# author-hidden-name/GAN-segmentation

Hardware: AMD Instinct MI355X
Metric: synthetic (image,mask) pairs/sec, FFHQ-1024 StyleGAN+decoder (higher is better)
Workload: dtype f32; 1 GPU; stylegan-ffhq 1024^2 synthesis + 2-class decoder, batch=8 per GPU, fp32 (BASELINE.json configs[1]); synthetic weights/latents/noise; (img u8, mask u8) resident on rank 0; global_batch=8, parallelism=dp1, gather=none, backend=none, graph=eager (GSA_GRAPH=0)

## Files before the change

### gan-segmentation_amd/csrc/gsa_api.cpp

```cpp
#include <hip/hip_runtime.h>

#include <cmath>
#include <cstdarg>
#include <cstdio>
#include <cstdlib>
#include <cstring>
#include <map>
#include <string>
#include <vector>

#include "../../include/gsa.h"
#include "gsa_kernels.h"
#include "gsa_pack.h"

using namespace gsa;

namespace {

constexpr int kMaxLevels = 12;
thread_local std::string g_create_error;

struct HostTensor {
    std::vector<float> data;
    std::vector<int64_t> dims;
// ... 213 lines not shown
}

bool known_generator_name(const gsa_ctx* c, const char* name) {
    int R = 0, k = 0, i = 0;
    char tail[64], t2[64];
    if (!strcmp(name, "constant_tensor") || !strcmp(name, "latent_avg") || !strcmp(name, "truncation_psi")) return true;
    if (sscanf(name, "mp_dense_%d_%63s", &i, tail) == 2)
        return i >= 0 && i < 8 && (!strcmp(tail, "weight") || !strcmp(tail, "bias") || !strcmp(tail, "std"));
    if (sscanf(name, "%d_%63s", &R, tail) != 2) return false;
    int r = 0;
    while ((1 << r) < R) ++r;
    if ((1 << r) != R || r < 2 || r > c->gc.max_res_log2) return false;
    if (!strcmp(tail, "conv_1_weight") || !strcmp(tail, "conv_1_std")) return r > 2 && r < 7;
    if (!strcmp(tail, "deconv_1_weight") || !strcmp(tail, "deconv_1_std")) return r >= 7;
    if (!strcmp(tail, "blur_1_w_kernel")) return r > 2;
    if (!strcmp(tail, "conv_2_weight") || !strcmp(tail, "conv_2_std")) return true;
    if (!strcmp(tail, "conv_to_rgb_weight") || !strcmp(tail, "conv_to_rgb_bias") || !strcmp(tail, "conv_to_rgb_std"))
        return r == c->gc.max_res_log2;
    if (sscanf(tail, "noise_%d_%63s", &k, t2) == 2) return (k == 1 || k == 2) && !strcmp(t2, "scale_factors");
    if (sscanf(tail, "bias_%d_%63s", &k, t2) == 2) return (k == 1 || k == 2) && !strcmp(t2, "bias");
    if (sscanf(tail, "adain_%d_%63s", &k, t2) == 2)
        return (k == 1 || k == 2) &&
               (!strcmp(t2, "dense_affine_weight") || !strcmp(t2, "dense_affine_bias") || !strcmp(t2, "dense_affine_std") ||
                !strcmp(t2, "norm_gamma") || !strcmp(t2, "norm_beta"));
    return false;
}

int set_param(gsa_ctx* c, std::map<std::string, HostTensor>& m, const char* name, const float* data, int ndim,
              const int64_t* dims) {
    if (!name || !data || ndim < 0 || ndim > 8) return fail(c, GSA_ERR_INVALID, "bad parameter tensor %s", name ? name : "(null)");
    HostTensor t;
    size_t cnt = 1;
    for (int i = 0; i < ndim; ++i) {
        if (dims[i] < 0) return fail(c, GSA_ERR_INVALID, "negative dimension in %s", name);
        t.dims.push_back(dims[i]);
        cnt *= (size_t)dims[i];
    }
    t.data.assign(data, data + cnt);
    m[name] = std::move(t);
    return GSA_OK;
}


struct Launch {
    gsa_ctx* c;
    hipStream_t s;
    const char* label;
    double flops, bytes, alg;
    std::string entry_layer;
    hipEvent_t a = nullptr;
    Launch(gsa_ctx* ctx, hipStream_t st, const char* layer, double flops_, double bytes_, double alg_ = -1.0)
        : c(ctx), s(st), label(layer), flops(flops_), bytes(bytes_), alg(alg_ < 0 ? flops_ : alg_) {
        (void)take_launch_record();
        if (!c->prof) return;
        if (c->prof > 1 && layer) entry_layer = layer;
        if (c->bf16 && layer && strncmp(layer, "g.mapping", 9) && strncmp(layer, "g.styles", 8) && !strstr(layer, "finalize")) bytes *= 0.5;
        a = event();
        (void)hipEventRecord(a, s);
    }
    hipEvent_t event() {
        if (c->event_pool.empty()) {
            hipEvent_t e = nullptr;
            (void)hipEventCreate(&e);
            return e;
        }
        hipEvent_t e = c->event_pool.back();
        c->event_pool.pop_back();
        return e;
    }
    ~Launch() {
        const LaunchRecord r = take_launch_record();
#ifdef GSA_STAMP
        const std::string kname_s = r.count == 1 ? kernel_name(r.kern) : std::string();
        const char* kname = kname_s.c_str();
        if (c->stamps && label && (strstr(kname, "conv") || strstr(kname, "subpixel"))) {
            (void)hipStreamSynchronize(s);
            unsigned long long h[16];
            (void)hipMemcpy(h, c->stamps, sizeof h, hipMemcpyDeviceToHost);
            (void)hipMemset(c->stamps, 0, sizeof h);
            if (h[15] && strstr(kname, "_ws")) {
                const double w = (double)h[15];
                fprintf(stderr, "STAMPWS %-24s %-16s waves %6llu  mfma: work %9.0f barrier %9.0f | mem: write %9.0f load %9.0f epi %9.0f barrier %9.0f\n",
                        kname, label, h[15], h[0] / w, h[1] / w, h[2] / w, h[3] / w, h[4] / w, h[5] / w);
            } else if (h[15] && h[8]) {
                const double w = (double)h[12];
                fprintf(stderr, "STAMPDB %-70s %-14s waves %6llu items/wave %5.1f | per item: write %6.0f load %6.0f (epi-loads %5.0f index %5.0f bulk %5.0f) mfma %6.0f epi %6.0f barrier %6.0f\n",
                        kname, label, h[15], h[12] / (double)h[15], h[6] / w, h[7] / w, h[0] / w, h[1] / w, h[2] / w, h[8] / w, h[9] / w, h[10] / w);
                if (strstr(kname, "subpixel"))
                    fprintf(stderr, "STAMPSW %-14s barrier by wave: %6.0f %6.0f %6.0f %6.0f | write wave0 %6.0f wave3 %6.0f\n", label, 4 * h[0] / w, 4 * h[1] / w, 4 * h[2] / w, 4 * h[3] / w, 4 * h[4] / w, 4 * h[5] / w);
            } else if (h[15]) {
                const double w = (double)h[15];
                fprintf(stderr, "STAMP %-40s %-16s waves %8llu  load %7.0f  write %6.0f  bar %6.0f  blocks %8.0f  epi %7.0f\n", kname,
                        label, h[15], h[0] / w, h[1] / w, h[2] / w, h[3] / w, h[4] / w);
            }
        }
#endif
        if (!a) return;
        if (r.count != 1) {
            c->event_pool.push_back(a);
            if (r.count > 1) ++c->prof_multi;
            return;
        }
        int entry = -1;
        for (size_t i = 0; i < c->prof_entries.size() && entry < 0; ++i)
            if (c->prof_entries[i].kern == r.kern && c->prof_entries[i].layer == entry_layer) entry = (int)i;
        if (entry < 0) {
            ProfEntry e;
            e.kern = r.kern;
            e.layer = entry_layer;
            c->prof_entries.push_back(e);
            entry = (int)c->prof_entries.size() - 1;
        }
        ProfEntry& e = c->prof_entries[entry];
        e.flops += flops;
        e.alg_flops += alg;
        e.bytes += bytes;
        e.launches += 1;
        hipEvent_t b = event();
        (void)hipEventRecord(b, s);
        c->prof_events.push_back(ProfEvent{a, b, entry});
    }
};

}


extern "C" {

#define GSA_STR2(x) #x
#define GSA_STR(x) GSA_STR2(x)
const char* gsa_version(void) {
#ifndef GSA_EXPERIMENTS
#define GSA_EXPERIMENTS 0
#endif
    return "gsa-hip 0.5"
#if GSA_EXPERIMENTS
           "+experiments"
#endif
           " (gfx950, v_mfma_f32_16x16x4_f32 implicit-GEMM convs; built with hipcc = clang " __clang_version__
           ", HIP " GSA_STR(HIP_VERSION_MAJOR) "." GSA_STR(HIP_VERSION_MINOR) "." GSA_STR(HIP_VERSION_PATCH) ")";
}

int gsa_create(int device, gsa_ctx** out) {
    if (!out) return fail(nullptr, GSA_ERR_INVALID, "gsa_create: out is null");
    int count = 0;
    hipError_t e = hipGetDeviceCount(&count);
    if (e != hipSuccess || count <= 0)
        return fail(nullptr, GSA_ERR_HIP, "no HIP device available (%s)", e == hipSuccess ? "device count is 0" : hipGetErrorString(e));
    if (device < 0 || device >= count) return fail(nullptr, GSA_ERR_INVALID, "device %d out of range (%d devices)", device, count);
    e = hipSetDevice(device);
    if (e != hipSuccess) return fail(nullptr, GSA_ERR_HIP, "hipSetDevice(%d): %s", device, hipGetErrorString(e));
    gsa_ctx* c = new gsa_ctx();
    c->device = device;
    e = hipStreamCreateWithFlags(&c->side, hipStreamNonBlocking);
    for (int i = 0; e == hipSuccess && i < kMaxLevels; ++i) e = hipEventCreateWithFlags(&c->ev_level[i], hipEventDisableTiming);
    if (e == hipSuccess) e = hipEventCreateWithFlags(&c->ev_fork, hipEventDisableTiming);
    if (e == hipSuccess) e = hipEventCreateWithFlags(&c->ev_join, hipEventDisableTiming);
    if (e != hipSuccess) {
        const int rc = fail(nullptr, GSA_ERR_HIP, "creating the side stream: %s", hipGetErrorString(e));
        delete c;
        return rc;
    }
    if (e == hipSuccess) e = hipMalloc((void**)&c->zeros, 256);
    if (e == hipSuccess) e = hipMemset(c->zeros, 0, 256);
    if (e != hipSuccess) {
        const int rc = fail(nullptr, GSA_ERR_HIP, "allocating the zero page: %s", hipGetErrorString(e));
// ... 866 lines not shown
```

### gan-segmentation_amd/csrc/gsa_kernels.h

```cpp
#pragma once
#include <hip/hip_runtime.h>
#include <stdint.h>
#include <stdlib.h>

#include <atomic>
#include <string>

namespace gsa {

struct Aff { float mean, A, B, pad; };

struct StatPart { unsigned long long s1, s2; };

constexpr double kStatScale1 = 268435456.0;

enum Epilogue { EPI_RAW = 0, EPI_SYNTH = 1, EPI_DEC = 2 };

struct ConvParams {
    int device;
    const float* src0; const Aff* aff0; int C0;
    const float* src1; int C1;
    int Hs, Ws;
    int up;
    int H, W;
    const float* wpk;
    const float* wino;
    int Cout;
    float* out;
    const float* noise; const float* nscale; const float* nbias;
    StatPart* partials; int prow;
    const float* bn_s; const float* bn_beta;
    const float* resid; int resid_up;
    const float* resid1; int res_c0;
    const float* wsc; const float* sc_bias; float* out_sc;
    int tiles_x, tiles_y, groups, total_tiles;
    int stats_direct;
    int* stat_rows_host;
    int w_resident;
    int group_minor;
    unsigned long long* stamps;
    int dbg;
    int prio;
    int bf16;
    const float* fin_style; int fin_style_stride; const float* fin_gamma; const float* fin_beta; Aff* fin_aff; unsigned* fin_flags;
    const float* zeros;
    const float* rgb_w; const float* rgb_b; uint8_t* rgb_img;
};

struct PostParams {
    const float* src;
    int src_per_sample;
    const float* blur;
    const float* noise; const float* nscale; const float* nbias;
    float* out; StatPart* partials; int prow;
    int H, W, C;
    int bf16;
    int row_groups;
};

struct FinalizeParams {
    const StatPart* partials; int prow; int HW; int C;
    StatPart* acc;
    unsigned* tickets;
    const float* style; int style_stride;
    const float* gamma; const float* beta;
    Aff* aff;
    unsigned* flags;
};

inline int env_int(const char* name, int dflt) {
    const char* v = getenv(name);
    return v ? atoi(v) : dflt;
}


enum class ConvForm { Wino43, WinoDma, WinoTwoTiles, WinoLean, Wino, KSplit, Bf16Lean, Direct };
ConvForm conv3x3_form(const ConvParams& p, int epi, bool shortcut);
hipError_t launch_conv3x3(const ConvParams& p, int epi, bool shortcut, int n, hipStream_t s);
inline bool conv_form_wino(ConvForm f) { return f <= ConvForm::Wino; }
inline double conv_form_products(ConvForm f) { return f == ConvForm::Wino43 ? 2.25 : conv_form_wino(f) ? 4 : 9; }
inline bool wino_shape(int H, int Cout, int bf16) { return !bf16 && (H >= 64 || (H >= 32 && Cout >= 64) || (H >= 16 && Cout >= 256)); }
inline bool wino43_shape(int H, int Cin) { return Cin >= 64 && H >= 32; }
bool wino43_enabled();
bool wino_lean_applies(const ConvParams& p, int epi);
bool wino_stream_paired(const ConvParams& p, int n);
hipError_t launch_wino_lean(const ConvParams& p, int epi, int n, hipStream_t s);
bool wino_lean_fuses_torgb(const ConvParams& p, int epi, int nc);
bool conv_fuses_torgb(const ConvParams& p, int epi, bool shortcut, int nc);
bool bf16_lean_applies(const ConvParams& p, int epi, bool shortcut);
hipError_t launch_bf16_lean(const ConvParams& p, int epi, int n, hipStream_t s);
bool subpixel_lean_applies(const ConvParams& p, int nt, int epi, bool sc, int kb, bool wst);
hipError_t launch_subpixel_lean(const ConvParams& q, int nt, int epi, bool sc, int kb, bool wst, dim3 grid, hipStream_t s);
enum class SubPath { Resident, Streamed, Plain };
struct SubpixelPlan {
    int ct;
    SubPath path;
    bool wino;
    int kb;
    size_t lds;
    int wgs_per_group;
};
SubpixelPlan subpixel_plan(const ConvParams& p, bool shortcut, int n);
hipError_t launch_subpixel(const ConvParams& p, int epi, bool shortcut, int n, hipStream_t s);
bool subpixel_uses_wino(const ConvParams& p);
enum class PostKind { Dma, Packed, Rows, OneRow };
struct PostPlan { PostKind kind; int rpt, row_groups, blocks, rows_used; };
PostPlan post_plan(const PostParams& p);
hipError_t launch_post(const PostParams& p, int n, hipStream_t s);
int post_pk_mode();
bool post_dma_applies(const PostParams& p);
int post_dma_band(const PostParams& p);
int post_dma_blocks(const PostParams& p);
hipError_t launch_post_dma(const PostParams& p, int n, hipStream_t s);
hipError_t launch_post_pk(const PostParams& q, dim3 grid, size_t lds, hipStream_t s);
hipError_t launch_finalize(const FinalizeParams& p, int n, hipStream_t s);
bool conv_fuses_finalize(const ConvParams& p, int epi, bool shortcut);
bool post_fuses_finalize(const PostParams& p);
hipError_t launch_post_fin(const PostParams& p, const FinalizeParams& f, int n, hipStream_t s);
hipError_t launch_pixelnorm(const float* z, float* out, int n, int L, hipStream_t s);
constexpr int kMapSlices = 8;
bool mapping_fused(int L, int device);
hipError_t launch_mapping(const float* z, float* const* wt, float* const* b, unsigned long long* const* ll, float* out, unsigned* ctl,
                          int n, int L, int device, hipStream_t s, int drop_workgroups = 0);
hipError_t launch_dense(const float* x, const float* WT, const float* b, float* y, int n, int K, int J,
                        int lrelu, hipStream_t s);
hipError_t launch_styles(const float* w, const float* avg, const float* psi, const float* WT, const float* b,
                         const int* col_layer, float* styles, int n, int K, int J, hipStream_t s);
hipError_t launch_styles_dlatents(const float* dlatents, const float* avg, const float* psi, const float* WT, const float* b,
                                  const int4* tiles, int num_tiles, float* styles, int n, int K, int J, int NL, hipStream_t s);
hipError_t launch_torgb(const float* x, const Aff* aff, const float* w, const float* b, float* rgb,
                        uint8_t* img, int n, int H, int W, int C, int nc, int bf16, hipStream_t s);
hipError_t launch_torgb_down(const float* x, const Aff* aff, const float* w, const float* b, uint8_t* img, int n, int H, int W, int C,
                             int nc, int f, int bf16, hipStream_t s);
hipError_t launch_final_conv_down(const float* src0, int C0, const float* src1, int C1, const float* wpk, const float* bias, uint8_t* mask,
                                  int n, int H, int W, int ncls, int f, int bf16, hipStream_t s);
hipError_t launch_export_nchw(const float* x, const Aff* aff, float* out, int n, int H, int W, int C, int bf16, hipStream_t s);
hipError_t launch_import_nhwc(const float* in, float* out, int n, int H, int W, int C, int bf16, hipStream_t s);
hipError_t launch_final_conv(const float* src0, int C0, const float* src1, int C1, const float* wpk,
                             const float* bias, float* logits, uint8_t* mask, int n, int H, int W, int ncls, int bf16,
                             hipStream_t s);

int conv_stat_rows(int H, int W, int Cout, int n);
int post_prow(int H, int W, int C);
int post_rows_used(const PostParams& p);
hipError_t launch_fill_normal(float* out, int per_sample, int n, unsigned long long first_index, unsigned plane,
                              unsigned long long seed, hipStream_t s);
hipError_t launch_seg_eval(const float* logits, const int8_t* labels, int n, int classes, int H, int W,
                           unsigned long long* confusion, unsigned long long* loss_fixed, hipStream_t s);

constexpr int kMaxDevices = 64;
int device_cus(int device);
int current_device();
hipError_t allow_max_lds(const void* kern);
hipError_t cached_occupancy(const void* kern, int device, int block, size_t lds, int* wgs_per_cu);
void note_launch(const void* kern);
struct LaunchRecord { const void* kern = nullptr; int count = 0; };
LaunchRecord take_launch_record();
std::string kernel_name(const void* kern);

template <auto K>
hipError_t prepare_kernel(int device) {
    static std::atomic<uint64_t> ready{0};
    if (device < 0 || device >= kMaxDevices) return hipErrorInvalidDevice;
    if (ready.load(std::memory_order_acquire) >> device & 1) return hipSuccess;
    if (hipError_t e = allow_max_lds(reinterpret_cast<const void*>(K))) return e;
    ready.fetch_or(1ull << device, std::memory_order_release);
    return hipSuccess;
}
// ... 17 lines not shown
```

### gan-segmentation_amd/csrc/gsa_wino_lean.hip

```cpp
#include "gsa_kernels.h"
#include "gsa_dev.h"

#include <cstdio>
#include <cstdlib>
#include <type_traits>

namespace gsa {
namespace lean {

constexpr int LH = 18, LW = 18, RS = LW * 16 + 4;
constexpr int IMG = LH * RS;
constexpr int SEG = 16 * 256;
constexpr int NPIX = LH * LW;

struct Tile { int n, y0, x0; };

template <int EPI, bool AFF, bool RES, int NB, int GW, bool DB = true, int PF = 1, bool RGB = false>
__global__ __launch_bounds__(256 * GW, GW == 1 ? (DB ? 2 : 3) : 1) void conv3x3_wino_lean(ConvParams p) {
    static_assert(!RGB || (NB == 1 && GW == 1 && DB && AFF && EPI == EPI_DEC), "fused toRGB: the 16 -> 16 decoder kernel with an AdaIN source");
    static_assert(DB || (NB == 1 && GW == 1), "single-buffered form: one block, one group");
    static_assert(PF == 1 || (PF == 2 && DB), "two prefetch sets: the double-buffered form");
    constexpr int NTHR = 256 * GW, CIN = 16 * NB, COUT = 16 * GW;
    constexpr int NCH = (NPIX * 4 + NTHR - 1) / NTHR;
    constexpr bool kLastPartial = (NPIX * 4) % NTHR != 0;
// ... 297 lines not shown
                epilogue(tc);
                if (EPI == EPI_SYNTH && (!has_next || tr.n != tc.n)) flush_stats(tc.n);
            }
            TICK(k4);
            __syncthreads();
            TICK(k5);
            TSUM(sw, k0, k1); TSUM(sl, k1, k2); TSUM(sm, k2, k3); TSUM(se, k3, k4); TSUM(sb, k4, k5);
            tc = tr; ec = er; cbc = cbr; tr = t2; er = e2c; cbr = cb2; t2 = t3; e2c = e3c; cb2 = cb3;
        };
        for (int it = 0; it < items; it += 2) {
            body(S1{}, it);
            if (it + 1 < items) body(S0{}, it + 1);
        }
        TFLUSH(6, sw); TFLUSH(7, sl); TFLUSH(8, sm); TFLUSH(9, se); TFLUSH(10, sb);
        TFLUSH(12, (unsigned long long)items); TFLUSH(15, 1ull);
        return;
    }
    if (items > 1) { next_item(tr, er, cbr); load_item(S0{}, tr, er, cbr); }
    loads_landed(ra[0]);
    __syncthreads();
    if constexpr (DB) {
        for (int it = 0; it < items; ++it) {
            const bool has_next = it + 1 < items;
            TICK(k0);
            if (has_next) write_item(S0{}, tr, er, cbr, (it + 1) & 1);
            TICK(k1);
            if (cbc == NB - 1) epilogue_loads(tc);
            Tile t2 = tr; int e2c = er, cb2 = cbr;
            if (it + 2 < items) { next_item(t2, e2c, cb2); load_item(S0{}, t2, e2c, cb2); }
            TICK(k2);
            if (NB == 1 || cbc == 0) multiply(std::true_type{}, it & 1, 0);
            else multiply(std::false_type{}, it & 1, cbc);
            loads_landed(ra[0], acc[15]);
            TICK(k3);
            if constexpr (RGB) torgb(tc, it & 1);
            if (cbc == NB - 1) {
                epilogue(tc);
                if (EPI == EPI_SYNTH && (!has_next || tr.n != tc.n)) flush_stats(tc.n);
            }
            TICK(k4);
            __syncthreads();
            TICK(k5);
            TSUM(sw, k0, k1); TSUM(sl, k1, k2); TSUM(sm, k2, k3); TSUM(se, k3, k4); TSUM(sb, k4, k5);
            tc = tr; ec = er; cbc = cbr; tr = t2; er = e2c; cbr = cb2;
        }
        TFLUSH(6, sw); TFLUSH(7, sl); TFLUSH(8, sm); TFLUSH(9, se); TFLUSH(10, sb);
        TFLUSH(12, (unsigned long long)items); TFLUSH(15, 1ull);
    } else {
        for (int it = 0; it < items; ++it) {
            const bool has_next = it + 1 < items;
            transform(0);
            __syncthreads();
            if (has_next) write_item(S0{}, tr, er, 0, 0);
            epilogue_loads(tc);
            Tile t2 = tr; int e2c = er, cb2 = 0;
            if (it + 2 < items) { next_item(t2, e2c, cb2); load_item(S0{}, t2, e2c, cb2); }
            mfmas(std::true_type{}, 0);
            loads_landed(ra[0], acc[15]);
            epilogue(tc);
            if (EPI == EPI_SYNTH && (!has_next || tr.n != tc.n)) flush_stats(tc.n);
            __syncthreads();
            tc = tr; ec = er; tr = t2; er = e2c;
        }
    }
}

__device__ unsigned g_cu_tickets[4096];
__device__ __forceinline__ void antiphase_start(int cycles64, float* lds_word) {
    if (cycles64 <= 0) return;
    if (threadIdx.x == 0) {
        unsigned hw, xcc;
        asm volatile("s_getreg_b32 %0, hwreg(HW_REG_HW_ID)" : "=s"(hw));
        asm volatile("s_getreg_b32 %0, hwreg(HW_REG_XCC_ID)" : "=s"(xcc));
        const unsigned cu = ((xcc & 15u) << 8) | (((hw >> 13) & 7u) << 5) | (((hw >> 12) & 1u) << 4) | ((hw >> 8) & 15u);
        *reinterpret_cast<unsigned*>(lds_word) = atomicAdd(&g_cu_tickets[cu & 4095u], 1u);
    }
    __syncthreads();
    const unsigned ticket = *reinterpret_cast<volatile unsigned*>(lds_word);
    __syncthreads();
    if (ticket & 1u)
        for (int i = 0; i < cycles64; i += 16) __builtin_amdgcn_s_sleep(16);
}

template <int EPI, bool AFF, int NT, int IL, bool PAIR>
__device__ __forceinline__ void wino_stream_body(const ConvParams& p) {
    static_assert(!PAIR || (NT == 1 && IL == 0), "paired form: one group per wave quad, phased memory instructions");
    constexpr int NTHR = PAIR ? 512 : 256;
    constexpr int NCH = (NPIX * 4 + NTHR - 1) / NTHR;
    constexpr int NP = PAIR ? 2 : NT;
    extern __shared__ __attribute__((aligned(16))) float smem[];
    float* const sA = smem;
    float* const sB = smem + 2 * IMG;
    float* const sE = sB + 2 * NP * SEG;
    float* const sC = sE + 64 * NP;
    const int tid = threadIdx.x, lane = tid & 63;
    const int wave8 = __builtin_amdgcn_readfirstlane(tid >> 6);
    const int wave = PAIR ? wave8 & 3 : wave8;
    const int quad = PAIR ? wave8 >> 2 : 0;
    const int i16 = lane & 15, kq = lane >> 4, part = tid & 3;
    const int H = p.H, W = p.W, CIN = p.C0, COUT = p.Cout, nblk = p.C0 >> 4;
    const int g = PAIR ? 2 * (int)blockIdx.y + quad : (int)blockIdx.y;
    const int per = (p.total_tiles + (int)gridDim.x - 1) / (int)gridDim.x;
    const int w_begin = xcd_block(blockIdx.x, gridDim.x) * per;
    const int w_end = min(p.total_tiles, w_begin + per);
    if (w_begin >= w_end) return;
    const int items = (w_end - w_begin) * nblk;
#if GSA_EXPERIMENTS
    antiphase_start(p.group_minor, sC);
#endif

    unsigned s_off[NCH], eflags = 0;
    int l_off[NCH];
#pragma unroll
    for (int k = 0; k < NCH; ++k) {
        const int pix = (tid + NTHR * k) >> 2;
        const bool real = pix < NPIX;
        const int ly = real ? pix / LW : 1, lx = real ? pix % LW : 1;
        s_off[k] = (unsigned)(((ly * W + lx) * CIN + part * 4) * 4);
        l_off[k] = real ? ly * RS + lx * 16 + part * 4 : -1;
        eflags |= (unsigned)((ly == 0 ? 1 : 0) | (ly == LH - 1 ? 2 : 0) | (lx == 0 ? 4 : 0) | (lx == LW - 1 ? 8 : 0)) << (4 * k);
    }
    const unsigned safe_off = (unsigned)((((W + 1) * CIN) + part * 4) * 4);
    auto edge_code = [&](const Tile& t) { return (t.y0 == 0 ? 1 : 0) | (t.y0 + 16 == H ? 2 : 0) | (t.x0 == 0 ? 4 : 0) | (t.x0 + 16 == W ? 8 : 0); };
    auto advance = [&](Tile& t) { t.x0 += 16; if (t.x0 == W) { t.x0 = 0; t.y0 += 16; if (t.y0 == H) { t.y0 = 0; t.n += 1; } } };

    f32x4 ra[NCH];
    int dbg_items = 0; (void)dbg_items;
    const float* const wgrp = p.wpk + (size_t)g * NT * nblk * SEG + lane * 4;
    auto dma_weights = [&](int cb, int buf) {
#ifdef GSA_DBG_HOOKS
        if (p.dbg & 16) cb = 0;
        if ((p.dbg & 1024) && dbg_items > 2) return;
#endif
#pragma unroll
        for (int ct = 0; ct < NT; ++ct) {
            const float* wb = wgrp + ((size_t)ct * nblk + cb) * SEG;
#pragma unroll
            for (int j = 0; j < 4; ++j) {
                const int piece = wave + 4 * j;
                __builtin_amdgcn_global_load_lds((const __attribute__((address_space(1))) void*)(wb + piece * 256),
                                                 (__attribute__((address_space(3))) void*)(sB + (PAIR ? buf * 2 + quad : buf * NT + ct) * SEG + piece * 256), 16, 0, 0);
            }
        }
    };
    auto load_item = [&](const Tile& t, int e, int cb) {
        const char* hb = reinterpret_cast<const char*>(p.src0) + ((((long)(t.n * H + t.y0) * W + t.x0) - (W + 1)) * CIN + cb * 16) * 4;
#ifdef GSA_DBG_HOOKS
        if (p.dbg & 32) hb = reinterpret_cast<const char*>(p.src0) + ((long)(W + 1) * CIN) * 4;
        if ((p.dbg & 512) && dbg_items > 2) return;
#endif
        if (e) {
#pragma unroll
            for (int k = 0; k < NCH; ++k) {
                const unsigned bad = (eflags >> (4 * k)) & (unsigned)e;
                const unsigned off = s_off[k] + (bad ? safe_off - s_off[k] : 0u);
                ra[k] = *reinterpret_cast<const f32x4*>(hb + off);
            }
        } else {
#pragma unroll
            for (int k = 0; k < NCH; ++k) ra[k] = *reinterpret_cast<const f32x4*>(hb + s_off[k]);
        }
    };
    int n_coef = -1;
    auto coefficients = [&](int n) {
        __syncthreads();
        for (int e = tid; e < CIN; e += NTHR) {
            const f32x4 a = *reinterpret_cast<const f32x4*>(p.aff0 + (size_t)n * CIN + e);
            sC[(e >> 4) * 32 + (e & 15)] = a[1];
            sC[(e >> 4) * 32 + 16 + (e & 15)] = a[2];
// ... 152 lines not shown
                    for (int ct = 0; ct < NT; ++ct) {
                        const int f = fb * 4 + j;
                        accs[ct][f] = __builtin_amdgcn_mfma_f32_16x16x4f32(u[ct][j][cg], V[f][cg], FIRST && cg == 0 ? f32x4{0.f, 0.f, 0.f, 0.f} : accs[ct][f], 0, 0, 0);
                    }
        }
        __builtin_amdgcn_s_setprio(0);
    };
    auto epilogue_ct = [&](const Tile& t, auto ct_tag) {
        constexpr int ct = decltype(ct_tag)::value;
        f32x4 (&acc)[16] = accs[ct];
        mfma_settle(acc);
        f32x4 s0[4], s1[4];
#pragma unroll
        for (int j = 0; j < 4; ++j) {
            s0[j] = add4(add4(acc[j], acc[4 + j]), acc[8 + j]);
            s1[j] = sub4(sub4(acc[4 + j], acc[8 + j]), acc[12 + j]);
        }
        f32x4 y[2][2];
        y[0][0] = add4(add4(s0[0], s0[1]), s0[2]); y[0][1] = sub4(sub4(s0[1], s0[2]), s0[3]);
        y[1][0] = add4(add4(s1[0], s1[1]), s1[2]); y[1][1] = sub4(sub4(s1[1], s1[2]), s1[3]);
        char* ob = reinterpret_cast<char*>(p.out) + (((long)(t.n * H + t.y0) * W + t.x0) * COUT + ct * 16) * 4;
        const float* sEc = sE + (PAIR ? quad : ct) * 64 + kq * 4;
        const f32x4 e0 = *reinterpret_cast<const f32x4*>(sEc), e1 = *reinterpret_cast<const f32x4*>(sEc + 16);
        const f32x4 e2 = *reinterpret_cast<const f32x4*>(sEc + 32), e3 = *reinterpret_cast<const f32x4*>(sEc + 48);
#pragma unroll
        for (int i = 0; i < 2; ++i)
#pragma unroll
            for (int j = 0; j < 2; ++j) {
                f32x4 v = y[i][j];
                if (EPI == EPI_DEC) v = lrelu4(fma4(v, e2, e3), k02);
                if (EPI == EPI_SYNTH) {
                    const f32x2 tlo = j == 0 ? pk_mul2_lo(e0.xy, nz[i]) : pk_mul2_hi(e0.xy, nz[i]);
                    const f32x2 thi = j == 0 ? pk_mul2_lo(e0.zw, nz[i]) : pk_mul2_hi(e0.zw, nz[i]);
                    v = lrelu4(add4(add4(v, f32x4{tlo.x, tlo.y, thi.x, thi.y}), e1), k02);
                    y[i][j] = v;
                }
#ifdef GSA_DBG_HOOKS
                if (!(p.dbg & 64))
#endif
                *reinterpret_cast<f32x4*>(ob + ((long)i * W + j) * COUT * 4 + out_off) = v;
            }
        if (EPI == EPI_SYNTH) {
            f32x4 ps[2], pq[2];
#pragma unroll
            for (int i = 0; i < 2; ++i) {
                ps[i] = add4(y[i][0], y[i][1]);
                const f32x2 a0 = pk_mul2(y[i][0].xy, y[i][0].xy), a1 = pk_mul2(y[i][0].zw, y[i][0].zw);
                const f32x2 b0 = pk_mul2(y[i][1].xy, y[i][1].xy), b1 = pk_mul2(y[i][1].zw, y[i][1].zw);
                pq[i] = add4(f32x4{a0.x, a0.y, a1.x, a1.y}, f32x4{b0.x, b0.y, b1.x, b1.y});
            }
#pragma unroll
            for (int c = 0; c < 4; ++c) {
                const float keep_s = odd ? ps[1][c] : ps[0][c], send_s = odd ? ps[0][c] : ps[1][c];
                const float keep_q = odd ? pq[1][c] : pq[0][c], send_q = odd ? pq[0][c] : pq[1][c];
                dI1[ct][c] += to_fixed(keep_s + dpp_quad<0xB1>(send_s), kStatScale1);
                dI2[ct][c] += to_fixed_sq(keep_q + dpp_quad<0xB1>(send_q), s2);
            }
        }
    };
    auto epilogue = [&](const Tile& t) {
        epilogue_ct(t, std::integral_constant<int, 0>{});
        if constexpr (NT == 2) epilogue_ct(t, std::integral_constant<int, 1>{});
    };

    Tile tc, tr;
    {
        const int tx = w_begin % p.tiles_x, r = w_begin / p.tiles_x;
        tc.x0 = tx * 16; tc.y0 = (r % p.tiles_y) * 16; tc.n = r / p.tiles_y;
    }
    int ec = edge_code(tc), er, cbc = 0, cbr = 0;
    auto next_item = [&](Tile& t, int& e, int& cb) {
        if (++cb == nblk) { cb = 0; advance(t); e = edge_code(t); }
    };
    dma_weights(0, 0);
    load_item(tc, ec, 0);
    write_item(tc, ec, 0, 0);
    tr = tc; er = ec;
    if (items > 1) {
        next_item(tr, er, cbr);
        load_item(tr, er, cbr);
    }
    __builtin_amdgcn_s_waitcnt(0x0F70);
    __syncthreads();
    unsigned long long k0 = 0, k1 = 0, k2 = 0, k3 = 0, k4 = 0, k5 = 0, sw = 0, sl = 0, sm = 0, se = 0, sb = 0;
    (void)k0; (void)k1; (void)k2; (void)k3; (void)k4; (void)k5; (void)sw; (void)sl; (void)sm; (void)se; (void)sb;
    for (int it = 0; it < items; ++it) {
        const bool has_next = it + 1 < items;
        TICK(k0);
        if (has_next) {
            if (!IL) dma_weights(cbr, (it + 1) & 1);
            write_item(tr, er, cbr, (it + 1) & 1);
        }
        TICK(k1);
        if (cbc == nblk - 1) epilogue_loads(tc);
        Tile t2 = tr; int e2c = er, cb2 = cbr;
        if (it + 2 < items) { next_item(t2, e2c, cb2); if (!IL) load_item(t2, e2c, cb2); }
        TICK(k2);
        auto vm0 = [&]() { if (IL == 1 && has_next) dma_weights(cbr, (it + 1) & 1); };
        auto vm1 = [&]() { if (IL == 1 && it + 2 < items) load_item(t2, e2c, cb2); };
        if (cbc == 0) multiply(std::true_type{}, it & 1, vm0, vm1);
        else multiply(std::false_type{}, it & 1, vm0, vm1);
        vmem_drained(accs[NT - 1][15]);
        TICK(k3);
        if (cbc == nblk - 1) {
            epilogue(tc);
            if (EPI == EPI_SYNTH && (!has_next || tr.n != tc.n)) flush_stats(tc.n);
        }
        TICK(k4);
        __syncthreads();
        TICK(k5);
        TSUM(sw, k0, k1); TSUM(sl, k1, k2); TSUM(sm, k2, k3); TSUM(se, k3, k4); TSUM(sb, k4, k5);
        tc = tr; ec = er; cbc = cbr; tr = t2; er = e2c; cbr = cb2;
    }
    TFLUSH(6, sw); TFLUSH(7, sl); TFLUSH(8, sm); TFLUSH(9, se); TFLUSH(10, sb);
    TFLUSH(12, (unsigned long long)items); TFLUSH(15, 1ull);
}

template <int EPI, bool AFF, int NT = 1, int IL = 0>
__global__ __launch_bounds__(256, NT == 1 ? 2 : 1) void conv3x3_wino_stream(ConvParams p) {
    wino_stream_body<EPI, AFF, NT, IL, false>(p);
}

template <int EPI, bool AFF>
__global__ __launch_bounds__(512, 1) void conv3x3_wino_stream_pair(ConvParams p) {
    wino_stream_body<EPI, AFF, 1, 0, true>(p);
}

template <int EPI, bool AFF, bool RES, int NB, int GW, bool DB = true, int PF = 1, bool RGB = false>
hipError_t launch_t(const ConvParams& p, int n, hipStream_t s) {
    const size_t lds = sizeof(float) * ((DB ? 2 : 1) * IMG + GW * NB * SEG);
    const int cus = device_cus(p.device);
    ConvParams q = p;
    q.wpk = p.wino;
    q.tiles_x = p.W / 16;
    q.tiles_y = p.H / 16;
    q.groups = 1;
    q.total_tiles = q.tiles_x * q.tiles_y * n;
    if (EPI == EPI_SYNTH) {
        q.stats_direct = 1;
        q.prow = kDirectRows;
        if (p.stat_rows_host) *p.stat_rows_host = q.prow;
    }
    const int gx = std::min(q.total_tiles, cus * (GW == 1 ? (DB ? 2 : 3) : 1));
    return launch<conv3x3_wino_lean<EPI, AFF, RES, NB, GW, DB, PF, RGB>>(p.device, dim3(gx), dim3(256 * GW), lds, s, q);
}

bool single_buffered() {
    static const bool on = env_int("GSA_WINO_LEAN_SB", 0) != 0;
    return on;
}

int prefetch_sets() {
    static const int pf = env_int("GSA_WINO_LEAN_PF", 1);
    return pf == 2 ? 2 : 1;
}

template <int NB, int GW>
hipError_t launch_shape(const ConvParams& p, int epi, int n, hipStream_t s) {
    if constexpr (NB == 1 && GW == 1) {
        if (epi == EPI_DEC && single_buffered()) {
            if (p.resid) return p.aff0 ? launch_t<EPI_DEC, true, true, 1, 1, false>(p, n, s) : launch_t<EPI_DEC, false, true, 1, 1, false>(p, n, s);
            return p.aff0 ? launch_t<EPI_DEC, true, false, 1, 1, false>(p, n, s) : launch_t<EPI_DEC, false, false, 1, 1, false>(p, n, s);
        }
    }
    if constexpr (NB == 1 && GW == 1) {
        if (p.rgb_img != nullptr) {
            if (epi != EPI_DEC || !p.aff0 || p.resid) return hipErrorInvalidValue;
            return launch_t<EPI_DEC, true, false, 1, 1, true, 1, true>(p, n, s);
        }
        if (prefetch_sets() == 2) {
            if (epi == EPI_DEC) {
                if (p.resid) return p.aff0 ? launch_t<EPI_DEC, true, true, 1, 1, true, 2>(p, n, s) : launch_t<EPI_DEC, false, true, 1, 1, true, 2>(p, n, s);
                return p.aff0 ? launch_t<EPI_DEC, true, false, 1, 1, true, 2>(p, n, s) : launch_t<EPI_DEC, false, false, 1, 1, true, 2>(p, n, s);
            }
            if (epi == EPI_SYNTH) return p.aff0 ? launch_t<EPI_SYNTH, true, false, 1, 1, true, 2>(p, n, s) : launch_t<EPI_SYNTH, false, false, 1, 1, true, 2>(p, n, s);
        }
    }
    if (epi == EPI_DEC) {
        if (p.resid) return p.aff0 ? launch_t<EPI_DEC, true, true, NB, GW>(p, n, s) : launch_t<EPI_DEC, false, true, NB, GW>(p, n, s);
        return p.aff0 ? launch_t<EPI_DEC, true, false, NB, GW>(p, n, s) : launch_t<EPI_DEC, false, false, NB, GW>(p, n, s);
    }
    if (epi == EPI_SYNTH) return p.aff0 ? launch_t<EPI_SYNTH, true, false, NB, GW>(p, n, s) : launch_t<EPI_SYNTH, false, false, NB, GW>(p, n, s);
    return hipErrorInvalidValue;
}

template <int EPI, bool AFF, int NT = 1, int IL = 0, bool PAIR = false>
hipError_t launch_stream_t(const ConvParams& p, int n, hipStream_t s) {
    constexpr int NP = PAIR ? 2 : NT;
    const int nblk = p.C0 / 16;
    const size_t lds = sizeof(float) * (2 * IMG + 2 * NP * SEG + 64 * NP + nblk * 32);
    const int cus = device_cus(p.device);
    ConvParams q = p;
    q.wpk = p.wino;
    q.tiles_x = p.W / 16;
    q.tiles_y = p.H / 16;
    q.groups = p.Cout / (16 * NP);
#if GSA_EXPERIMENTS
    static const int stagger = env_int("GSA_STAGGER", 0);
    q.group_minor = PAIR ? 0 : stagger;
#else
    q.group_minor = 0;
#endif
    q.total_tiles = q.tiles_x * q.tiles_y * n;
    if (EPI == EPI_SYNTH) {
        q.stats_direct = 1;
        q.prow = kDirectRows;
        if (p.stat_rows_host) *p.stat_rows_host = q.prow;
    }
    const int slots = std::max(1, cus * (NP == 1 ? 2 : 1) / q.groups);
    const int gx = std::min(q.total_tiles, slots);
    if constexpr (PAIR) return launch<conv3x3_wino_stream_pair<EPI, AFF>>(p.device, dim3(gx, q.groups), dim3(512), lds, s, q);
    else return launch<conv3x3_wino_stream<EPI, AFF, NT, IL>>(p.device, dim3(gx, q.groups), dim3(256), lds, s, q);
}

}
using namespace lean;

bool wino_lean_applies(const ConvParams& p, int epi) {
    static const int enabled = env_int("GSA_WINO_LEAN", 7);
    if (p.H != p.W || p.H % 16) return false;
    if ((enabled & 4) && p.C0 >= 64 && p.C0 <= 512 && p.resid == nullptr && p.H >= 16)
        return epi == EPI_SYNTH ? (p.partials != nullptr && p.noise != nullptr && p.fin_aff == nullptr) : epi == EPI_DEC;
    const bool shape = (p.C0 == 16 && p.Cout == 16 && (enabled & 1)) || (p.C0 == 32 && p.Cout == 32 && (enabled & 2));
    if (!shape || p.H < 32) return false;
    if (epi == EPI_SYNTH) return p.partials != nullptr && p.noise != nullptr && p.fin_aff == nullptr && p.resid == nullptr;
    if (epi != EPI_DEC) return false;
    if (p.resid != nullptr && (p.resid_up != 1 || p.resid1 != nullptr)) return false;
    return true;
}

bool wino_lean_fuses_torgb(const ConvParams& p, int epi, int nc) {
    static const bool enabled = env_int("GSA_FUSE_RGB", 1) != 0;
    return enabled && nc == 3 && epi == EPI_DEC && p.C0 == 16 && p.Cout == 16 && p.aff0 != nullptr && p.resid == nullptr && !p.bf16 &&
           wino_lean_applies(p, epi) && !single_buffered();
}

bool wino_stream_paired(const ConvParams& p, int n) {
    static const int mode = env_int("GSA_WINO_PAIR", 1);
    if (mode <= 0 || p.C0 < 64 || p.Cout % 32) return false;
    if (mode == 2) return true;
    return (long)(p.W / 16) * (p.H / 16) * n * (p.Cout / 32) >= device_cus(p.device);
}

bool stream_pairs(const ConvParams& p, int n) {
#if GSA_EXPERIMENTS
    static const int on = env_int("GSA_WINO_NT2", 0);
    if (!on || p.Cout % 32) return false;
    const long wgs = (long)(p.W / 16) * (p.H / 16) * n * (p.Cout / 32);
    return wgs >= (on == 2 ? 1 : 256);
#else
    (void)p; (void)n;
    return false;
#endif
}

int stream_interleaved() {
#if GSA_EXPERIMENTS
    static const int il = env_int("GSA_WINO_IL", 0);
    return il == 1 ? 1 : 0;
#else
    return 0;
#endif
}

hipError_t launch_wino_lean(const ConvParams& p, int epi, int n, hipStream_t s) {
    if (p.C0 >= 64) {
#if GSA_EXPERIMENTS
        if (stream_pairs(p, n)) {
            const int il = stream_interleaved();
#define GSA_STREAM2(IL_) \
            if (il == IL_) { \
                if (epi == EPI_SYNTH) return p.aff0 ? launch_stream_t<EPI_SYNTH, true, 2, IL_>(p, n, s) : launch_stream_t<EPI_SYNTH, false, 2, IL_>(p, n, s); \
                if (epi == EPI_DEC) return p.aff0 ? launch_stream_t<EPI_DEC, true, 2, IL_>(p, n, s) : launch_stream_t<EPI_DEC, false, 2, IL_>(p, n, s); \
                return hipErrorInvalidValue; \
            }
            GSA_STREAM2(0) GSA_STREAM2(1)
#undef GSA_STREAM2
            return hipErrorInvalidValue;
        }
#endif
        if (wino_stream_paired(p, n)) {
            if (epi == EPI_SYNTH) return p.aff0 ? launch_stream_t<EPI_SYNTH, true, 1, 0, true>(p, n, s) : launch_stream_t<EPI_SYNTH, false, 1, 0, true>(p, n, s);
            if (epi == EPI_DEC) return p.aff0 ? launch_stream_t<EPI_DEC, true, 1, 0, true>(p, n, s) : launch_stream_t<EPI_DEC, false, 1, 0, true>(p, n, s);
            return hipErrorInvalidValue;
        }
        if (epi == EPI_SYNTH) return p.aff0 ? launch_stream_t<EPI_SYNTH, true>(p, n, s) : launch_stream_t<EPI_SYNTH, false>(p, n, s);
        if (epi == EPI_DEC) return p.aff0 ? launch_stream_t<EPI_DEC, true>(p, n, s) : launch_stream_t<EPI_DEC, false>(p, n, s);
        return hipErrorInvalidValue;
    }
    if (p.C0 == 16 && p.Cout == 16) return launch_shape<1, 1>(p, epi, n, s);
    if (p.C0 == 32 && p.Cout == 32) return launch_shape<2, 2>(p, epi, n, s);
    return hipErrorInvalidValue;
}

}
```

Before: 1422 pairs/s.

## Run second wave quad of paired Winograd stream kernel with opposed phase order

Adds an opposed-phase variant of the paired Winograd streaming conv kernel. In it, the second wave quad issues its weight DMA and epilogue loads before the multiply and its tile write and next-load after, so the two quads in a workgroup hit memory and MFMA at different times. The variant is enabled by default only for synthesis convs at 64x64x256 and 128x128x128 with enough workgroups. It adds a separate kernel instantiation and an early endpgm exit for the second quad, and relies on the barrier counts of the two loop bodies still matching.

Measured after the change: 1424 pairs/s, median of 6. No clear change (+0.1%).

```diff
diff --git a/gan-segmentation_amd/csrc/gsa_api.cpp b/gan-segmentation_amd/csrc/gsa_api.cpp
--- a/gan-segmentation_amd/csrc/gsa_api.cpp
+++ b/gan-segmentation_amd/csrc/gsa_api.cpp
@@ -319,6 +319,10 @@
                 const double w = (double)h[15];
                 fprintf(stderr, "STAMPWS %-24s %-16s waves %6llu  mfma: work %9.0f barrier %9.0f | mem: write %9.0f load %9.0f epi %9.0f barrier %9.0f\n",
                         kname, label, h[15], h[0] / w, h[1] / w, h[2] / w, h[3] / w, h[4] / w, h[5] / w);
+            } else if (h[15] && h[8] && strstr(kname, "stream_pair")) {
+                const double w = (double)h[12] / 2;
+                fprintf(stderr, "STAMPPQ %-70s %-14s waves %6llu items/wave %5.1f | per item, quad 0: write %6.0f load %6.0f mfma %6.0f epi %6.0f barrier %6.0f | quad 1: write %6.0f load %6.0f mfma %6.0f epi %6.0f barrier %6.0f\n",
+                        kname, label, h[15], h[12] / (double)h[15], h[6] / w, h[7] / w, h[8] / w, h[9] / w, h[10] / w, h[0] / w, h[1] / w, h[2] / w, h[3] / w, h[4] / w);
             } else if (h[15] && h[8]) {
                 const double w = (double)h[12];
                 fprintf(stderr, "STAMPDB %-70s %-14s waves %6llu items/wave %5.1f | per item: write %6.0f load %6.0f (epi-loads %5.0f index %5.0f bulk %5.0f) mfma %6.0f epi %6.0f barrier %6.0f\n",
diff --git a/gan-segmentation_amd/csrc/gsa_kernels.h b/gan-segmentation_amd/csrc/gsa_kernels.h
--- a/gan-segmentation_amd/csrc/gsa_kernels.h
+++ b/gan-segmentation_amd/csrc/gsa_kernels.h
@@ -84,6 +84,7 @@
 bool wino43_enabled();
 bool wino_lean_applies(const ConvParams& p, int epi);
 bool wino_stream_paired(const ConvParams& p, int n);
+bool wino_pair_opposed(const ConvParams& p, int epi, int n);
 hipError_t launch_wino_lean(const ConvParams& p, int epi, int n, hipStream_t s);
 bool wino_lean_fuses_torgb(const ConvParams& p, int epi, int nc);
 bool conv_fuses_torgb(const ConvParams& p, int epi, bool shortcut, int nc);
diff --git a/gan-segmentation_amd/csrc/gsa_wino_lean.hip b/gan-segmentation_amd/csrc/gsa_wino_lean.hip
--- a/gan-segmentation_amd/csrc/gsa_wino_lean.hip
+++ b/gan-segmentation_amd/csrc/gsa_wino_lean.hip
@@ -403,9 +403,10 @@
         for (int i = 0; i < cycles64; i += 16) __builtin_amdgcn_s_sleep(16);
 }
 
-template <int EPI, bool AFF, int NT, int IL, bool PAIR>
+template <int EPI, bool AFF, int NT, int IL, bool PAIR, bool OPP = false>
 __device__ __forceinline__ void wino_stream_body(const ConvParams& p) {
     static_assert(!PAIR || (NT == 1 && IL == 0), "paired form: one group per wave quad, phased memory instructions");
+    static_assert(!OPP || PAIR, "opposed phase order: the two quads of the paired form");
     constexpr int NTHR = PAIR ? 512 : 256;
     constexpr int NCH = (NPIX * 4 + NTHR - 1) / NTHR;
     constexpr int NP = PAIR ? 2 : NT;
@@ -724,8 +725,46 @@
     }
     __builtin_amdgcn_s_waitcnt(0x0F70);
     __syncthreads();
-    unsigned long long k0 = 0, k1 = 0, k2 = 0, k3 = 0, k4 = 0, k5 = 0, sw = 0, sl = 0, sm = 0, se = 0, sb = 0;
-    (void)k0; (void)k1; (void)k2; (void)k3; (void)k4; (void)k5; (void)sw; (void)sl; (void)sm; (void)se; (void)sb;
+    unsigned long long k0 = 0, k1 = 0, k2 = 0, k3 = 0, k4 = 0, k5 = 0, k6 = 0, k7 = 0, sw = 0, sl = 0, sm = 0, se = 0, sb = 0;
+    (void)k0; (void)k1; (void)k2; (void)k3; (void)k4; (void)k5; (void)k6; (void)k7; (void)sw; (void)sl; (void)sm; (void)se; (void)sb;
+    auto flush_stamps = [&]() {
+        const int sq = PAIR && quad ? 0 : 6; (void)sq;
+        TFLUSH(sq, sw); TFLUSH(sq + 1, sl); TFLUSH(sq + 2, sm); TFLUSH(sq + 3, se); TFLUSH(sq + 4, sb);
+        TFLUSH(12, (unsigned long long)items); TFLUSH(15, 1ull);
+    };
+    const bool opposed = OPP && quad != 0;
+    if constexpr (OPP) { if (opposed) {
+        for (int it = 0; it < items; ++it) {
+            const bool has_next = it + 1 < items;
+                TICK(k0);
+                if (has_next) dma_weights(cbr, (it + 1) & 1);
+                TICK(k1);
+                if (cbc == nblk - 1) epilogue_loads(tc);
+                TICK(k2);
+                auto none = [&]() {};
+                if (cbc == 0) multiply(std::true_type{}, it & 1, none, none);
+                else multiply(std::false_type{}, it & 1, none, none);
+                vmem_drained(accs[NT - 1][15]);
+                TICK(k3);
+                if (cbc == nblk - 1) {
+                    epilogue(tc);
+                    if (EPI == EPI_SYNTH && (!has_next || tr.n != tc.n)) flush_stats(tc.n);
+                }
+                TICK(k4);
+                if (has_next) write_item(tr, er, cbr, (it + 1) & 1);
+                TICK(k5);
+                Tile t2 = tr; int e2c = er, cb2 = cbr;
+                if (it + 2 < items) { next_item(t2, e2c, cb2); load_item(t2, e2c, cb2); }
+                TICK(k6);
+                __syncthreads();
+                TICK(k7);
+                TSUM(sw, k0, k1); TSUM(sl, k1, k2); TSUM(sm, k2, k3); TSUM(se, k3, k4); TSUM(sw, k4, k5); TSUM(sl, k5, k6); TSUM(sb, k6, k7);
+            tc = tr; ec = er; cbc = cbr; tr = t2; er = e2c; cbr = cb2;
+        }
+        flush_stamps();
+        __builtin_amdgcn_endpgm();
+    } }
+    if constexpr (OPP) __builtin_amdgcn_s_waitcnt(0x0F70);
     for (int it = 0; it < items; ++it) {
         const bool has_next = it + 1 < items;
         TICK(k0);
@@ -754,8 +793,7 @@
         TSUM(sw, k0, k1); TSUM(sl, k1, k2); TSUM(sm, k2, k3); TSUM(se, k3, k4); TSUM(sb, k4, k5);
         tc = tr; ec = er; cbc = cbr; tr = t2; er = e2c; cbr = cb2;
     }
-    TFLUSH(6, sw); TFLUSH(7, sl); TFLUSH(8, sm); TFLUSH(9, se); TFLUSH(10, sb);
-    TFLUSH(12, (unsigned long long)items); TFLUSH(15, 1ull);
+    flush_stamps();
 }
 
 template <int EPI, bool AFF, int NT = 1, int IL = 0>
@@ -766,6 +804,11 @@
 template <int EPI, bool AFF>
 __global__ __launch_bounds__(512, 1) void conv3x3_wino_stream_pair(ConvParams p) {
     wino_stream_body<EPI, AFF, 1, 0, true>(p);
+}
+
+template <int EPI, bool AFF>
+__global__ __launch_bounds__(512, 1) void conv3x3_wino_stream_pair_opp(ConvParams p) {
+    wino_stream_body<EPI, AFF, 1, 0, true, true>(p);
 }
 
 template <int EPI, bool AFF, bool RES, int NB, int GW, bool DB = true, int PF = 1, bool RGB = false>
@@ -826,7 +869,7 @@
     return hipErrorInvalidValue;
 }
 
-template <int EPI, bool AFF, int NT = 1, int IL = 0, bool PAIR = false>
+template <int EPI, bool AFF, int NT = 1, int IL = 0, bool PAIR = false, bool OPP = false>
 hipError_t launch_stream_t(const ConvParams& p, int n, hipStream_t s) {
     constexpr int NP = PAIR ? 2 : NT;
     const int nblk = p.C0 / 16;
@@ -851,7 +894,8 @@
     }
     const int slots = std::max(1, cus * (NP == 1 ? 2 : 1) / q.groups);
     const int gx = std::min(q.total_tiles, slots);
-    if constexpr (PAIR) return launch<conv3x3_wino_stream_pair<EPI, AFF>>(p.device, dim3(gx, q.groups), dim3(512), lds, s, q);
+    if constexpr (PAIR && OPP) return launch<conv3x3_wino_stream_pair_opp<EPI, AFF>>(p.device, dim3(gx, q.groups), dim3(512), lds, s, q);
+    else if constexpr (PAIR) return launch<conv3x3_wino_stream_pair<EPI, AFF>>(p.device, dim3(gx, q.groups), dim3(512), lds, s, q);
     else return launch<conv3x3_wino_stream<EPI, AFF, NT, IL>>(p.device, dim3(gx, q.groups), dim3(256), lds, s, q);
 }
 
@@ -884,6 +928,14 @@
     return (long)(p.W / 16) * (p.H / 16) * n * (p.Cout / 32) >= device_cus(p.device);
 }
 
+bool wino_pair_opposed(const ConvParams& p, int epi, int n) {
+    static const int mode = env_int("GSA_PAIR_PHASE", 1);
+    if (mode <= 0 || !wino_stream_paired(p, n)) return false;
+    if (mode >= 2) return true;
+    if (epi != EPI_SYNTH || (long)(p.W / 16) * (p.H / 16) * n * (p.Cout / 32) < device_cus(p.device)) return false;
+    return (p.H == 64 && p.C0 == 256 && p.Cout == 256) || (p.H == 128 && p.C0 == 128 && p.Cout == 128);
+}
+
 bool stream_pairs(const ConvParams& p, int n) {
 #if GSA_EXPERIMENTS
     static const int on = env_int("GSA_WINO_NT2", 0);
@@ -922,6 +974,11 @@
         }
 #endif
         if (wino_stream_paired(p, n)) {
+            if (wino_pair_opposed(p, epi, n)) {
+                if (epi == EPI_SYNTH) return p.aff0 ? launch_stream_t<EPI_SYNTH, true, 1, 0, true, true>(p, n, s) : launch_stream_t<EPI_SYNTH, false, 1, 0, true, true>(p, n, s);
+                if (epi == EPI_DEC) return p.aff0 ? launch_stream_t<EPI_DEC, true, 1, 0, true, true>(p, n, s) : launch_stream_t<EPI_DEC, false, 1, 0, true, true>(p, n, s);
+                return hipErrorInvalidValue;
+            }
             if (epi == EPI_SYNTH) return p.aff0 ? launch_stream_t<EPI_SYNTH, true, 1, 0, true>(p, n, s) : launch_stream_t<EPI_SYNTH, false, 1, 0, true>(p, n, s);
             if (epi == EPI_DEC) return p.aff0 ? launch_stream_t<EPI_DEC, true, 1, 0, true>(p, n, s) : launch_stream_t<EPI_DEC, false, 1, 0, true>(p, n, s);
             return hipErrorInvalidValue;
```
